# WagnerGroup/pyqmc

Measured on AMD Instinct MI355X. Metric: walker-steps/sec (VMC sweep, 64e- Slater-Jastrow), higher is better.
Workload: dtype f64

## Files before the change

### pyqmc_amd/csrc/pqa_ao.hpp

```cpp
#pragma once
#include "pqa_common.hpp"
#include "pqa_sph_high.hpp"

__device__ __forceinline__ double exp_neg(double x) {
  x = fmax(x, -800.0);
  const double k = __builtin_rint(x * 1.4426950408889634074);
  double r = fma(-k, 6.93147180369123816490e-01, x);
  r = fma(-k, 1.90821492927058770002e-10, r);
  double p = 2.519062899249436e-08;
  p = fma(p, r, 2.761249479944321e-07);
  p = fma(p, r, 2.7557019442003614e-06);
  p = fma(p, r, 2.480153911822949e-05);
  p = fma(p, r, 0.0001984127010654779);
  p = fma(p, r, 0.0013888888904182626);
  p = fma(p, r, 0.008333333333235474);
  p = fma(p, r, 0.04166666666665442);
  p = fma(p, r, 0.1666666666666677);
  p = fma(p, r, 0.5);
  p = fma(p, r, 1.0);
  p = fma(p, r, 1.0);
  return ldexp(p, (int)k);
}
__device__ __forceinline__ void exp_neg3(double x0, double x1, double x2, double& e0, double& e1, double& e2) {
  x0 = fmax(x0, -800.0); x1 = fmax(x1, -800.0); x2 = fmax(x2, -800.0);
// ... 35 lines not shown
#define SH_F3 0.5900435899266435
#define SH_F2 2.890611442640554
#define SH_F1 0.4570457994644658
#define SH_F0 0.3731763325901154
#define SH_F2C 1.445305721320277

__device__ __forceinline__ double sph_ipow(double x, int n) {
  double r = 1.0;
#pragma unroll 1
  for (int q = 0; q < n; ++q) r *= x;
  return r;
}
__device__ __forceinline__ void sph_high(int l, int m, double x, double y, double z, double& s, double& sx, double& sy, double& sz) {
  s = sx = sy = sz = 0.0;
  const int t1 = SPH_HI_OFF[l - 4][m + 1];
#pragma unroll 1
  for (int t = SPH_HI_OFF[l - 4][m]; t < t1; ++t) {
    const SphTerm q = SPH_HI_TERM[t];
    const double xa = sph_ipow(x, q.i - 1), ya = sph_ipow(y, q.j - 1), za = sph_ipow(z, q.k - 1);
    const double xi = q.i ? xa * x : 1.0, yj = q.j ? ya * y : 1.0, zk = q.k ? za * z : 1.0;
    s += q.c * xi * yj * zk;
    if (q.i) sx += q.c * q.i * xa * yj * zk;
    if (q.j) sy += q.c * q.j * xi * ya * zk;
    if (q.k) sz += q.c * q.k * xi * yj * za;
  }
}

#define PQA_RT_X0 0.0078125
#define PQA_RT_NSUB 8
#define PQA_RT_DEG 9
#define PQA_RT_REC (PQA_RT_DEG + 1)
#define PQA_RT_MINP 3
#define PQA_RT_MAXERR 2e-15
__device__ __forceinline__ double radial_tab(const double* __restrict__ tab, int nint, double r2) {
  const double y = r2 + PQA_RT_X0;
  const int E = __builtin_amdgcn_frexp_exp(y);
  const double m = __builtin_amdgcn_frexp_mant(y);
  const double t = fma(m, 2.0 * PQA_RT_NSUB, -(double)PQA_RT_NSUB);
  const double tj = floor(t);
  const double u = fma(t - tj, 2.0, -1.0);
  int idx = (E + 6) * PQA_RT_NSUB + (int)tj;
  const bool in = idx < nint;
  idx = in ? idx : nint - 1;
  const double2* rec = reinterpret_cast<const double2*>(tab + (size_t)idx * PQA_RT_REC);
  double c[PQA_RT_REC];
#pragma unroll
  for (int q = 0; q < PQA_RT_REC / 2; ++q) { const double2 v = rec[q]; c[2 * q] = v.x; c[2 * q + 1] = v.y; }
  double f0 = c[PQA_RT_DEG];
#pragma unroll
  for (int q = PQA_RT_DEG - 1; q >= 0; --q) f0 = fma(f0, u, c[q]);
  return in ? f0 : 0.0;
}
template <int NCOMP, int LMAX = 5, class Sink>
__device__ __forceinline__ void shell_angular(int l, double x, double y, double z, double R, double dRs, double lapR, Sink&& sink);
template <int NCOMP, int LMAX = 5, bool SCREEN = false, class Sink>
__device__ __forceinline__ void shell_eval(int l, double x, double y, double z, const double* __restrict__ pexp,
                                           const double* __restrict__ pcoef, int np, Sink&& sink) {
  const double r2 = x * x + y * y + z * z;
  double R = 0.0, dRs = 0.0, lapR = 0.0;
#pragma unroll 1
  for (int p = 0; p < np; ++p) {
    const double a = pexp[p];
    if (SCREEN && a * r2 > PQA_PRIM_CUT) continue;
    const double t = pcoef[p] * exp_neg(-a * r2);
    R += t;
    if (NCOMP > 1) dRs += a * t;
    if (NCOMP == 5) lapR += t * (2.0 * a) * (2.0 * a * r2 - 3.0);
  }
  shell_angular<NCOMP, LMAX>(l, x, y, z, R, dRs, lapR, sink);
}
template <int LMAX = 5, class Sink>
__device__ __forceinline__ void shell_eval_tab(int l, double x, double y, double z, const double* __restrict__ tab, int nint, Sink&& sink) {
  shell_angular<1, LMAX>(l, x, y, z, radial_tab(tab, nint, x * x + y * y + z * z), 0.0, 0.0, sink);
}
template <int NCOMP, int LMAX = 5, class Sink>
__device__ __forceinline__ void shell_eval3(int l, double x, double y, double z, const double* __restrict__ pexp,
                                            const double* __restrict__ pcoef, int np, Sink&& sink) {
  const double r2 = x * x + y * y + z * z;
  double R = 0.0, dRs = 0.0, lapR = 0.0;
  auto add = [&](double a, double c, double e) __attribute__((always_inline)) {
    const double t = c * e;
    R += t;
    if (NCOMP > 1) dRs += a * t;
    if (NCOMP == 5) lapR += t * (2.0 * a) * (2.0 * a * r2 - 3.0);
// ... 459 lines not shown
  const double* a = ao + ((size_t)c * P + p) * nao;
  double s = 0.0;
  for (int k = 0; k < nao; ++k) s += a[k] * C[(size_t)k * nmo + j];
  out[(sel ? (size_t)(sel[p] ^ 1) * slot_stride : (size_t)0) + ((size_t)p * ncomp + c) * nmo + j] = s;
}

template <int PQA_UNIT = 0>
static __global__ void k_mo_valu(const double* __restrict__ ao, const double* __restrict__ C, long rows, int nao, int nmo,
                          double* __restrict__ out) {
  const long idx = (long)blockIdx.x * blockDim.x + threadIdx.x;
  if (idx >= rows * nmo) return;
  const long r = idx / nmo;
  const int j = idx % nmo;
  double s = 0.0;
  for (int a = 0; a < nao; ++a) s += ao[r * nao + a] * C[(long)a * nmo + j];
  out[idx] = s;
}

struct ChunkTab {
  int nchunk;
  const int* chunk_nk;
  const int* shell_kb;
  const int* chunk_row0;
  const int* cw_off[3];
  const int* cw_shell[3];
  const double* cpad[2];
  int ldc[2];
  int col0;
  const double* pbc_d0;
  const unsigned long long* pbc_list;
  int pbc_nw;
  const unsigned char* out_sel;
  long out_slot_stride;
};
__device__ __forceinline__ double* orb_out(const ChunkTab& T, double* out, long p) {
  return T.out_sel ? out + (size_t)(T.out_sel[p] ^ 1) * T.out_slot_stride : out;
}

#define PQA_LS_MAX 128
#define PQA_WS_MAXSH 160
#define PQA_WS_MAXP 640

template <int NCOMP, int NT, int KC, int TP, bool LDSTAB, int PBC = 0>
static __global__ __launch_bounds__(256) void k_orb(SysDev S, ChunkTab T, int spin, PointAddr pa, long P,
                                             double* __restrict__ out) {
  P = point_count(pa, P);
  if ((long)blockIdx.x * TP >= P) return;
  constexpr int G = 256 / TP;
  constexpr int NU = (TP == 64) ? NT : ((TP == 32) ? (NT + 1) / 2 : (NT + 3) / 4);
  constexpr int KS = KC / 4;
  __shared__ double tile[NCOMP][KC][TP];
  __shared__ double sh_xyz[LDSTAB ? PQA_WS_MAXSH : 1][3];
  __shared__ int sh_meta[LDSTAB ? PQA_WS_MAXSH : 1][7];
  __shared__ double pr_exp[LDSTAB ? PQA_WS_MAXP : 1], pr_coef[LDSTAB ? PQA_WS_MAXP : 1];
  __shared__ double sh_Ls[PBC ? PQA_LS_MAX : 1][3], sh_ph[PBC == 2 ? PQA_LS_MAX : 1][2];
  const int tid = threadIdx.x, lane = tid & 63, wv = tid >> 6;
  const bool ls_lds = PBC && S.nL <= PQA_LS_MAX;
  if (PBC && ls_lds) {
    for (int q = tid; q < 3 * S.nL; q += 256) sh_Ls[q / 3][q % 3] = S.pb->Ls[q];
    if (PBC == 2) for (int q = tid; q < 2 * S.nL; q += 256) sh_ph[q / 2][q % 2] = S.pb->img_phase[q];
    if (!LDSTAB) __syncthreads();
  }
  if (LDSTAB) {
    for (int sh = tid; sh < S.nshell; sh += 256) {
      const int ia = S.shell_atom[sh];
      sh_xyz[sh][0] = S.atom_xyz[3 * ia]; sh_xyz[sh][1] = S.atom_xyz[3 * ia + 1]; sh_xyz[sh][2] = S.atom_xyz[3 * ia + 2];
// ... 413 lines not shown
```

### pyqmc_amd/csrc/pqa_create.hip

```cpp
#include "pqa_internal.hpp"

static thread_local std::string g_create_error;

static double det3(const double* a) { return a[0] * (a[4] * a[8] - a[5] * a[7]) - a[1] * (a[3] * a[8] - a[5] * a[6]) + a[2] * (a[3] * a[7] - a[4] * a[6]); }
static void inv3(const double* a, double det, double* v) {
  const double id = 1.0 / det;
  v[0] = (a[4] * a[8] - a[5] * a[7]) * id; v[1] = (a[2] * a[7] - a[1] * a[8]) * id; v[2] = (a[1] * a[5] - a[2] * a[4]) * id;
  v[3] = (a[5] * a[6] - a[3] * a[8]) * id; v[4] = (a[0] * a[8] - a[2] * a[6]) * id; v[5] = (a[2] * a[3] - a[0] * a[5]) * id;
  v[6] = (a[3] * a[7] - a[4] * a[6]) * id; v[7] = (a[1] * a[6] - a[0] * a[7]) * id; v[8] = (a[0] * a[4] - a[1] * a[3]) * id;
}

static int member_masks(pqa_handle* h, const pqa_system_t* sys, PbcDev& P) {
  P.memb_mask = nullptr;
  P.memb_E = 0;
  const int side = 2 * sys->member_M + 1, E = side, T = side + 2 * E, nc = sys->n_member_class, nj = std::min(sys->nL, 128);
  if ((size_t)nc * T * T * T * 16 > ((size_t)64 << 20)) return 0;
  std::vector<unsigned char> mem((size_t)nc * side * side * side);
  std::vector<int> imgn((size_t)sys->nL * 3);
  HIPCHK(hipMemcpy(mem.data(), sys->member, mem.size(), hipMemcpyDefault));
  HIPCHK(hipMemcpy(imgn.data(), sys->img_n, imgn.size() * sizeof(int), hipMemcpyDefault));
  for (int j = 0; j < nj; ++j)
    for (int c = 0; c < 3; ++c)
      if (std::abs(imgn[3 * j + c]) > E) return 0;
  std::vector<unsigned long long> mask((size_t)nc * T * T * T * 2, 0ull);
// ... 264 lines not shown
      c.cw_off[0].push_back((int)c.cw_shell[0].size());
    }
    std::stable_sort(members.begin(), members.end(), [&](int a, int b) { return cost(a) > cost(b); });
    std::vector<std::vector<int>> l8(8);
    std::vector<int> load8(8, 0);
    for (int s : members) {
      int best = 0;
      for (int q = 1; q < 8; ++q)
        if (load8[q] < load8[best]) best = q;
      l8[best].push_back(s);
      load8[best] += cost(s);
    }
    for (int q = 0; q < 8; ++q) {
      for (int s : l8[q]) c.cw_shell[1].push_back(s);
      c.cw_off[1].push_back((int)c.cw_shell[1].size());
    }
    std::vector<std::vector<int>> l16(16);
    std::vector<int> load16(16, 0);
    for (int s : members) {
      int best = 0;
      for (int q = 1; q < 16; ++q)
        if (load16[q] < load16[best]) best = q;
      l16[best].push_back(s);
      load16[best] += cost(s);
    }
    for (int q = 0; q < 16; ++q) {
      for (int s : l16[q]) c.cw_shell[2].push_back(s);
      c.cw_off[2].push_back((int)c.cw_shell[2].size());
    }
  }
  c.rows_pad = row0;
}

static int upload_cpad(pqa_handle* h, int t, int s, const double* mo_host) {
  const ChunkHost& c = h->chunks[t];
  const int ldc = 16 * h->nt[s], nmo = h->nmo[s];
  std::vector<double> pad((size_t)std::max(c.rows_pad, 1) * ldc, 0.0);
  for (int sh = 0; sh < h->nshell; ++sh)
    for (int m = 0; m < 2 * h->shell_l[sh] + 1; ++m)
      for (int j = 0; j < nmo; ++j)
        pad[(size_t)(c.row0[c.shell_chunk[sh]] + c.shell_kb[sh] + m) * ldc + j] = mo_host[(size_t)(h->shell_ao[sh] + m) * nmo + j];
  if (h->twist) {
    const int nr = nmo / 2;
    for (int sh = 0; sh < h->nshell; ++sh) {
      const int sx = sh + h->nshell;
      for (int m = 0; m < 2 * h->shell_l[sh] + 1; ++m)
        for (int j = 0; j < nr; ++j) {
          const double* src = mo_host + (size_t)(h->shell_ao[sh] + m) * nmo;
          double* dst = pad.data() + (size_t)(c.row0[c.shell_chunk[sx]] + c.shell_kb[sx] + m) * ldc;
          dst[j] = -src[nr + j];
          dst[nr + j] = src[j];
        }
    }
  }
  HIPCHK(hipMemcpy(h->d_cpad[t][s], pad.data(), pad.size() * sizeof(double), hipMemcpyHostToDevice));
  return 0;
}

int set_mo(pqa_handle* h, int s, const double* mo_host) {
  if (h->nmo[s] == 0 || !mo_host) return 0;
  HIPCHK(hipMemcpy(h->d_mo[s], mo_host, (size_t)h->nao * std::max(h->nmo[s], 1) * sizeof(double), hipMemcpyHostToDevice));
  for (int t = 0; t < 2; ++t) TRY(upload_cpad(h, t, s, mo_host));
  TRY(cres_upload(h, s, mo_host));
  return 0;
}

// ... 213 lines not shown
      if (!(fabs(det) > 1e-12)) FAIL("singular primitive lattice");
      inv3(a, det, P.lprim_inv);
      const size_t side = 2 * (size_t)sys->member_M + 1;
      unsigned char* tmp_b;
      TRY(upload_table(h, sys->member, (size_t)sys->n_member_class * side * side * side, &tmp_b)); P.member = tmp_b;
      TRY(upload_table(h, sys->member_class, (size_t)h->natom, &tmp_i)); P.member_class = tmp_i;
      TRY(upload_table(h, sys->img_n, (size_t)sys->nL * 3, &tmp_i)); P.img_n = tmp_i;
      TRY(upload_table(h, sys->atom_n, (size_t)h->natom * 3, &tmp_i)); P.atom_n = tmp_i;
      P.member_M = sys->member_M;
      TRY(member_masks(h, sys, P));
      for (int i = 0; i < 9; ++i) {
        double v_ = 0.0;
        for (int k = 0; k < 3; ++k) v_ += sys->lattice[3 * (i / 3) + k] * P.lprim_inv[3 * k + (i % 3)];
        P.supercell[i] = (int)lround(v_);
        if (fabs(v_ - P.supercell[i]) > 1e-6) FAIL("lattice is not an integer multiple of lattice_prim");
      }
    }
  }
  return 0;
}

static int create_determinants(pqa_handle* h, const pqa_system_t* sys) {
  SysDev& S = h->S;
  int* tmp_i;
  h->nmo[0] = sys->nmo_up; h->nmo[1] = sys->nmo_dn;
  h->ndet = sys->ndet; h->ndet_s[0] = sys->ndet_up; h->ndet_s[1] = sys->ndet_dn;
  S.ndet = h->ndet;
  const int* occ_src[2] = {sys->det_occ_up, sys->det_occ_dn};
  const double* mo_src[2] = {sys->mo_up, sys->mo_dn};
  const int nel[2] = {h->nup, h->ndn};
  shell_costs(h, sys);
  build_chunks(h, 16, h->chunks[0]);
  build_chunks(h, 32, h->chunks[1]);
  for (int s = 0; s < 2; ++s) {
    if (h->nmo[s] > (h->cplx ? 2 : 1) * PQA_MAXN) FAIL("more than 128 orbitals per spin are not supported");
    const int nt = (h->nmo[s] + 15) / 16;
    h->nt[s] = nt <= 1 ? 1 : (nt == 2 ? 2 : (nt <= 4 ? 4 : (nt <= 8 ? 8 : 16)));
    S.nmo[s] = h->nmo[s]; S.ndet_s[s] = h->ndet_s[s];
    TRY(upload_table(h, occ_src[s], (size_t)h->ndet_s[s] * nel[s], &tmp_i)); S.det_occ[s] = tmp_i;
    {
      std::vector<int> oc((size_t)std::max(nel[s], 1));
      if (nel[s] > 0) HIPCHK(hipMemcpy(oc.data(), occ_src[s], (size_t)nel[s] * sizeof(int), hipMemcpyDefault));
      S.occ_ident[s] = 1;
      for (int k = 0; k < nel[s]; ++k) S.occ_ident[s] &= (oc[k] == k) ? 1 : 0;
    }
    {
      std::vector<int> occ_h((size_t)h->ndet_s[s] * nel[s]), cm((size_t)h->ndet_s[s] * std::max(h->nmo[s], 1), -1);
      if (!occ_h.empty()) HIPCHK(hipMemcpy(occ_h.data(), occ_src[s], occ_h.size() * sizeof(int), hipMemcpyDefault));
      for (int u = 0; u < h->ndet_s[s]; ++u)
        for (int k = 0; k < nel[s]; ++k) {
          const int m = occ_h[(size_t)u * nel[s] + k];
          if (m < 0 || m >= h->nmo[s]) FAIL("determinant occupation outside the orbital range");
          cm[(size_t)u * h->nmo[s] + m] = k;
        }
      TRY(upload_table(h, cm.data(), cm.size(), &h->d_colmap[s]));
    }
    TRY(upload_table<double>(h, nullptr, (size_t)h->nao * std::max(h->nmo[s], 1), &h->d_mo[s])); S.mo[s] = h->d_mo[s];
    for (int t = 0; t < 2; ++t)
      TRY(upload_table<double>(h, nullptr, (size_t)(std::max(h->chunks[t].rows_pad, 1) + 32) * 16 * h->nt[s], &h->d_cpad[t][s]));
    if (h->nmo[s] > 0) TRY(set_mo(h, s, mo_src[s]));
  }
  TRY(upload_table(h, sys->det_coeff, (size_t)h->ndet, &h->d_detcoeff)); S.det_coeff = h->d_detcoeff;
  TRY(upload_table(h, sys->det_map, (size_t)2 * h->ndet, &tmp_i)); S.det_map = tmp_i;
  for (int t = 0; t < 2; ++t) {
    const ChunkHost& c = h->chunks[t];
    ChunkTab& T = h->tab[t];
// ... 256 lines not shown
```

### pyqmc_amd/csrc/pqa_ecp_orbcol.hpp

```cpp
#pragma once
#include "pqa_ao.hpp"
#include "pqa_ecp.hpp"

#define PQA_OC_R 16
#define PQA_OC_KC 32
#define PQA_OC_STATIC_LDS ((size_t)PQA_WS_MAXSH * (3 * sizeof(double) + 6 * sizeof(int)) + (size_t)PQA_WS_MAXP * 2 * sizeof(double) + 4 * 64 * sizeof(double) + 2 * 64 * sizeof(int))
__host__ __device__ inline size_t ecp_orbcol_lds(int nao, int n) { return (size_t)PQA_OC_R * ((size_t)(nao | 1) + (size_t)((n + PQA_OC_KC - 1) / PQA_OC_KC * PQA_OC_KC)) * sizeof(double); }

static __global__ __launch_bounds__(256) void k_ecp_orbcol(SysDev S, LwState L, ChunkTab T, int s, PointAddr pa, long P, const int* __restrict__ pte,
                                                    const int* __restrict__ ptw, long W, double* __restrict__ ratio) {
  P = point_count(pa, P);
  const long p0 = (long)blockIdx.x * 64;
  if (p0 >= P) return;
  extern __shared__ __align__(16) double oc_lds[];
  __shared__ double sh_xyz[PQA_WS_MAXSH][3];
  __shared__ int sh_meta[PQA_WS_MAXSH][6];
  __shared__ double pr_exp[PQA_WS_MAXP], pr_coef[PQA_WS_MAXP];
  __shared__ double part[4][64];
  __shared__ int run_i[64], run_w[64];
  const int tid = threadIdx.x, lane = tid & 63, wv = __builtin_amdgcn_readfirstlane(tid >> 6);
  const int n = s ? S.ndn : S.nup, nmo = S.nmo[s], nao = S.nao, vs = nao | 1, nk = (n + PQA_OC_KC - 1) / PQA_OC_KC * PQA_OC_KC;
  const int* __restrict__ occ = S.det_occ[s];
  const bool ident = S.occ_ident[s] != 0;
  const double* __restrict__ Cs = S.mo[s];
  double c[PQA_OC_KC];
  auto load_row = [&](int mu, int k0) {
    const double* __restrict__ crow = Cs + (size_t)mu * nmo;
    if (ident && (nmo & 3) == 0 && k0 + PQA_OC_KC <= n) {
#pragma unroll
      for (int u = 0; u < PQA_OC_KC; u += 4) {
        const double4 q = *reinterpret_cast<const double4*>(crow + k0 + u);
        c[u] = q.x; c[u + 1] = q.y; c[u + 2] = q.z; c[u + 3] = q.w;
      }
    } else {
#pragma unroll
      for (int u = 0; u < PQA_OC_KC; ++u) {
        const int k = k0 + u;
        c[u] = (k < n) ? crow[ident ? k : occ[k]] : 0.0;
      }
    }
  };
  bool have_c = tid < nao;
  if (have_c) load_row(tid, 0);
  const bool c_stays = nao <= 256 && n <= PQA_OC_KC;
  for (int sh = tid; sh < S.nshell; sh += 256) {
    const int ia = S.shell_atom[sh];
    sh_xyz[sh][0] = S.atom_xyz[3 * ia]; sh_xyz[sh][1] = S.atom_xyz[3 * ia + 1]; sh_xyz[sh][2] = S.atom_xyz[3 * ia + 2];
    sh_meta[sh][0] = S.shell_l[sh];
    sh_meta[sh][1] = S.shell_prim_off[sh + 1] - S.shell_prim_off[sh];
    sh_meta[sh][2] = S.shell_prim_off[sh];
    sh_meta[sh][3] = S.shell_ao_off[sh];
    sh_meta[sh][4] = S.shell_rt[2 * sh]; sh_meta[sh][5] = S.shell_rt[2 * sh + 1];
  }
  for (int p = tid; p < S.nprim; p += 256) { pr_exp[p] = S.prim_exp[p]; pr_coef[p] = S.prim_coef[p]; }
  const long pmine = (p0 + lane < P) ? p0 + lane : P - 1;
  double px, py, pz;
  load_point(pa, pmine, px, py, pz);
  const int e = pte[pmine], w = ptw[pmine];
  const int e_prev = __shfl_up(e, 1, 64), w_prev = __shfl_up(w, 1, 64);
  const bool head = lane == 0 || e != e_prev || w != w_prev;
  const unsigned long long heads = __ballot(head);
  const int run = __popcll(heads & (~0ull >> (63 - lane))) - 1, nrun = __popcll(heads);
  if (wv == 0 && head) { run_i[run] = e - s * S.nup; run_w[run] = w; }
  double* V = oc_lds;
  double* tc = oc_lds + (size_t)PQA_OC_R * vs;
  const double* __restrict__ Tt = L.Tt[s];
  const int* __restrict__ cw_off = T.cw_off[0];
  const int* __restrict__ cw_shell = T.cw_shell[0];
  double acc = 0.0;
  for (int r0 = 0; r0 < nrun; r0 += PQA_OC_R) {
    const int nr = (nrun - r0 < PQA_OC_R) ? nrun - r0 : PQA_OC_R;
    __syncthreads();
    for (int idx = tid; idx < nk * PQA_OC_R; idx += 256) {
      const int k = idx / PQA_OC_R, r = idx % PQA_OC_R;
      tc[idx] = (r < nr && k < n) ? Tt[((size_t)run_i[r0 + r] * n + k) * W + run_w[r0 + r]] : 0.0;
    }
    __syncthreads();
    for (int mu = tid; mu < nao; mu += 256) {
      double v[PQA_OC_R];
#pragma unroll
      for (int r = 0; r < PQA_OC_R; ++r) v[r] = 0.0;
      for (int k0 = 0; k0 < nk; k0 += PQA_OC_KC) {
        if (!(have_c && mu == tid && k0 == 0)) load_row(mu, k0);
        if (!c_stays) have_c = false;
#pragma unroll
        for (int g = 0; g < PQA_OC_R; g += 4) {
          if (g < nr) {
#pragma unroll
            for (int u = 0; u < PQA_OC_KC; ++u) {
              const double4 t = *reinterpret_cast<const double4*>(tc + (k0 + u) * PQA_OC_R + g);
              v[g] = fma(c[u], t.x, v[g]); v[g + 1] = fma(c[u], t.y, v[g + 1]); v[g + 2] = fma(c[u], t.z, v[g + 2]); v[g + 3] = fma(c[u], t.w, v[g + 3]);
            }
          }
        }
      }
#pragma unroll
      for (int g = 0; g < PQA_OC_R; g += 4)
        if (g < nr) { V[g * vs + mu] = v[g]; V[(g + 1) * vs + mu] = v[g + 1]; V[(g + 2) * vs + mu] = v[g + 2]; V[(g + 3) * vs + mu] = v[g + 3]; }
    }
    __syncthreads();
    const bool mine = run >= r0 && run < r0 + nr;
    const double* __restrict__ Vr = V + (mine ? run - r0 : 0) * vs;
    double a = 0.0;
    for (int ch = 0; ch < T.nchunk; ++ch) {
      const int s_end = cw_off[ch * 4 + wv + 1];
      for (int si = cw_off[ch * 4 + wv]; si < s_end; ++si) {
        const int sh = cw_shell[si];
        const int l_ = __builtin_amdgcn_readfirstlane(sh_meta[sh][0]), np_ = __builtin_amdgcn_readfirstlane(sh_meta[sh][1]);
        const int q0 = __builtin_amdgcn_readfirstlane(sh_meta[sh][2]), row = __builtin_amdgcn_readfirstlane(sh_meta[sh][3]);
        const int rt_ = __builtin_amdgcn_readfirstlane(sh_meta[sh][4]), rn_ = __builtin_amdgcn_readfirstlane(sh_meta[sh][5]);
        const double x = px - sh_xyz[sh][0], y = py - sh_xyz[sh][1], z = pz - sh_xyz[sh][2];
        auto to_sum = [&](int m, double v, double, double, double, double) { a = fma(v, Vr[row + m], a); };
        if (rt_ >= 0) shell_eval_tab(l_, x, y, z, S.rtab + rt_, rn_, to_sum);
        else shell_eval<1>(l_, x, y, z, pr_exp + q0, pr_coef + q0, np_, to_sum);
      }
    }
    if (mine) acc = a;
  }
  part[wv][lane] = acc;
  __syncthreads();
  if (wv == 0 && p0 + lane < P) ratio[p0 + lane] = ((part[0][lane] + part[1][lane]) + part[2][lane]) + part[3][lane];
}
```

### pyqmc_amd/csrc/pqa_energy.hip

```cpp
#include "pqa_internal.hpp"
#include "pqa_ecp_orbcol.hpp"

namespace {

struct EnergyPlan {
  long W = 0;
  bool soa = false;
  bool has_jastrow = false, has_j2 = false;
  bool rot_tape = false, unif_tape = false;
  enum Kinetic { kin_lw, kin_coulomb } kinetic = kin_coulomb;
  bool kin_quad = false;
  int waves = 1;
  enum Coords { coords_none, coords_sweep, coords_transpose, coords_state } coords = coords_none;
  bool soa_T = false;
  bool ewald_planes = false;
  bool ecp = false;
  enum Lists { lists_none, lists_batched, lists_lds, lists_first } lists = lists_none;
  long nseg = 1;
  size_t tab_b = 0;
  long pmax = 0;
  bool scan_small = true;
  bool fill_ue = false;
  enum Orbitals { orb_none, orb_column, orb_rows } orbitals = orb_none;
  enum Points { pts_none, pts_point_lw, pts_point, pts_accum } points = pts_none;
// ... 270 lines not shown
    TRY(ensure(h, h->b_eptw[s], n * sizeof(int)));
    TRY(ensure(h, h->b_econ[s], (h->cplx ? 2 : 1) * n * sizeof(double)));
    TRY(ensure(h, h->b_eu0[s], n * sizeof(double)));
    B.ptw[s] = (int*)h->b_eptw[s].p;
    B.u0[s] = (double*)h->b_eu0[s].p;
    if (P.orbitals == EnergyPlan::orb_column) TRY(ensure(h, h->b_erat[s], n * sizeof(double)));
    else TRY(ensure(h, h->b_emo[s], n * std::max(h->nmo[s], 1) * sizeof(double)));
    B.pts[s] = (double*)h->b_epts[s].p; B.wgt[s] = (double*)h->b_ewgt[s].p; B.pte[s] = (int*)h->b_epte[s].p;
  }
  if (batched) {
    launch_ecpb_fill(h, B, A, W);
    TRY(check_launch(h, "k_ecpb_fill"));
  }
  if (P.soa) TRY(R.side.join());
  if (batched || R.tot[0] + R.tot[1] <= 0) return 0;
  if (P.lists == EnergyPlan::lists_lds)
    hipLaunchKernelGGL(ecp_fill_t_kernels[ix(P.fill_ue)][ix(h->S.pbc)], dim3((unsigned)((W + PQA_ECP_WB - 1) / PQA_ECP_WB)), dim3(64 * PQA_ECP_WB), P.tab_b,
                       h->stream, h->S, h->js, B, h->ecp_nchan, h->ecp_nterm, W);
  else
    hipLaunchKernelGGL(ecp_fill_kernels[ix(h->S.pbc)], dim3((unsigned)W), dim3(64), 0, h->stream, h->S, h->js, B, W);
  return check_launch(h, P.lists == EnergyPlan::lists_lds ? "k_ecp_fill_t" : "k_ecp_fill");
}

int stage_ecp_orbitals(EnergyRun& R) {
  pqa_handle* h = R.h;
  const EnergyPlan& P = R.P;
  if (R.tot[0] + R.tot[1] <= 0 || P.orbitals == EnergyPlan::orb_none) return 0;
  for (int s = 0; s < 2; ++s) {
    PointAddr pa = plain_points(R.B.pts[s], R.tot[s]);
    if (P.defer) pa.count = R.cnt_dev[s];
    if (P.orbitals == EnergyPlan::orb_column) {
      if (R.tot[s] <= 0 || h->nmo[s] == 0) continue;
      hipLaunchKernelGGL((k_ecp_orbcol), dim3((unsigned)((R.tot[s] + 63) / 64)), dim3(256), ecp_orbcol_lds(h->S.nao, s ? h->ndn : h->nup), h->stream,
                         h->S, lw_state(h), h->tab[1], s, pa, R.tot[s], (const int*)R.B.pte[s], (const int*)R.B.ptw[s], P.W, (double*)h->b_erat[s].p);
    } else {
      if (P.defer) h->orb_p_hint = std::max<long>(h->en.hint[s], 1);
      const int rc = launch_orb(h, s, pa, R.tot[s], 1, (double*)h->b_emo[s].p);
      h->orb_p_hint = 0;
      if (rc != 0) return rc;
    }
  }
  return P.orbitals == EnergyPlan::orb_column ? check_launch(h, "k_ecp_orbcol") : 0;
}

using EcpAccumKernel = void (*)(SysDev, SlaterState, JastrowState, EcpBuf, int, int, const double*, const double*, long, double*, int);
using EcpPointLwKernel = void (*)(SysDev, LwState, EcpBuf, int, int, int, const double*, long, long, double*, const double*, long, double*, const double*, const double*);
using EcpPointKernel = void (*)(SysDev, SlaterState, JastrowState, EcpBuf, int, int, int, const double*, long, double*, const double*, long, long, long);
const EcpAccumKernel ecp_accum_cx_kernels[2][2] = {
    {k_ecp_accum<true, true, 4>, k_ecp_accum<true, true, 1>}, {k_ecp_accum<false, true, 4>, k_ecp_accum<false, true, 1>}};
const EcpPointLwKernel ecp_point_lw_kernels[2][2] = {
    {k_ecp_point_lw<true, true>, k_ecp_point_lw<false, true>}, {k_ecp_point_lw<true, false>, k_ecp_point_lw<false, false>}};
const EcpPointKernel ecp_point_kernels[2] = {k_ecp_point<true>, k_ecp_point<false>};

int ecp_points(EnergyRun& R) {
  pqa_handle* h = R.h;
  const EnergyPlan& P = R.P;
  const EcpBuf& B = R.B;
  const long W = P.W;
  const long* tot = R.tot;
  const bool lw = P.points == EnergyPlan::pts_point_lw, column = P.orbitals == EnergyPlan::orb_column;
  const bool both = lw && tot[0] > 0 && tot[1] > 0 && std::max(h->en.hint[0], h->en.hint[1]) <= 262144 && h->en.hint_valid;
  for (int s = 0; s < 2; ++s) {
    if (tot[s] <= 0 || (both && s == 1)) continue;
    const int o = both ? 1 : s;
    const long n = both ? std::max(tot[0], tot[1]) : tot[s];
    const dim3 g((unsigned)((n + 255) / 256), both ? 2 : 1);
    if (lw)
// ... 165 lines not shown
    if (lds <= 64 * 1024) {
      int* dgi;
      TRY(upload_table(h, gi.data(), gi.size(), &dgi));
      h->ew.gn = dgi; h->ew.nmax = nmax;
      HIPCHK(hipMemcpy(h->ew.recip, recip, 9 * sizeof(double), hipMemcpyDefault));
    }
  }
  h->ii_energy = ii;
  h->ew_set = true;
  return 0;
}

extern "C" int pqa_get_wrap(pqa_handle_t* h, int32_t* wrap) {
  HIPCHK(hipSetDevice(h->device));
  if (!h->S.pbc) FAIL("open-boundary handle has no wrap counters");
  if (h->wrap_W != h->W || h->W == 0) FAIL("no fused sweep has run on the resident walkers");
  return copy_out(h, wrap, h->b_wrap.p, (size_t)h->W * h->N * 3 * sizeof(int));
}

extern "C" int pqa_energy(pqa_handle_t* h, double threshold, const double* rot, const double* unif, uint64_t seed, double* out) {
  TRY(sync_aos(h));
  HIPCHK(hipSetDevice(h->device));
  if (h->W == 0) FAIL("state not initialised (call pqa_wf_recompute)");
  h->saved_valid = false;
  TRY(energy_dev(h, threshold, rot, unif, seed, 0u));
  return copy_out(h, out, h->b_en.p, (size_t)(h->cplx ? 7 : 6) * h->W * sizeof(double));
}

extern "C" int pqa_energy_last(pqa_handle_t* h, double* out) {
  HIPCHK(hipSetDevice(h->device));
  if (h->W == 0 || h->en.W != h->W) FAIL("no energy evaluation has run on the resident walkers");
  return copy_out(h, out, h->b_en.p, (size_t)(h->cplx ? 7 : 6) * h->W * sizeof(double));
}
```

### pyqmc_amd/csrc/pqa_internal.hpp

```cpp
#pragma once
#include <hip/hip_runtime.h>

#include <algorithm>
#include <array>
#include <cmath>
#include <cstdio>
#include <cstdlib>
#include <cstring>
#include <string>
#include <vector>

#include "../../include/pyqmc_amd.h"
#include "pqa_ao.hpp"
#include "pqa_common.hpp"
#include "pqa_cslater.hpp"
#include "pqa_dmc.hpp"
#include "pqa_energy.hpp"
#include "pqa_ecp.hpp"
#include "pqa_ecpb.hpp"
#include "pqa_jastrow.hpp"
#include "pqa_lw.hpp"
#include "pqa_slater.hpp"
#include "pqa_res.hpp"
#include "pqa_res8_tab.hpp"
// ... 30 lines not shown
  std::vector<hipEvent_t> events;
  std::vector<hipStream_t> streams;
  std::vector<void*> pinned;
  int natom = 0, nup = 0, ndn = 0, N = 0, nao = 0, nshell = 0;
  int nmo[2] = {0, 0}, nt[2] = {1, 1}, ndet = 1, ndet_s[2] = {1, 1};
  int na = 0, nb = 0, necp = 0;
  bool aos_stale = false;
  int pbc_maxcls = PQA_PRE_NCUT;
  int pbc_nw = 2;
  bool orb_general = false;
  bool dmc_continue = false, dmc_old_valid = false;
  long dmc_old_W = 0;
  bool invert_attr = false;
  bool big = false;
  bool pbc_high_l = false;
  bool twist = false;
  bool cplx = false;
  bool has_slater = false, has_jastrow = false;
  bool has_j2 = false, has_j3 = false;
  int na3 = 0, nb3 = 0;
  double* d_c3 = nullptr;
  DevBuf b_j3u;
  double ii_energy = 0.0;
  EwaldDev ew{};
  bool ew_set = false;
  std::vector<int> shell_l, shell_np, shell_ao;
  int lmax = 0;
  std::vector<int> rt_shells;
  double rt_err = 0.0;
  std::vector<int> shell_cost;
  SysDev S{};
  ChunkHost chunks[2];
  ChunkTab tab[2]{};
  const unsigned char* out_sel = nullptr;
  long out_slot_stride = 0;
  int orb_col0 = 0;
  double* d_mo[2] = {nullptr, nullptr};
  double* d_cpad[2][2] = {{nullptr, nullptr}, {nullptr, nullptr}};
  double *d_acoeff = nullptr, *d_bcoeff = nullptr, *d_detcoeff = nullptr, *d_quad = nullptr, *d_quadw = nullptr;
  int *d_ecp_naip = nullptr, *d_ecp_qoff = nullptr;
  int ecp_naip = 0;
  std::vector<int> ecp_nch;
  int ecpb_on = 0, ecpb_npoints = 0, ecpb_nsd = 0, ecpb_nsr = 0, ecpb_nsel = 0;
  int *d_ecpb_naip = nullptr, *d_ecpb_qoff = nullptr, *d_ecpb_pstart = nullptr;
  double *d_aq = nullptr, *d_bq = nullptr;
  int jas_merge = 1;
  long W = 0;
  SlaterState st{};
  JastrowState js{};
  DevBuf b_x, b_T[2], b_dsign[2], b_dlog[2], b_cache[2], b_aval, b_bval;
  DevBuf b_alt_x, b_alt_T[2], b_alt_dsign[2], b_alt_dlog[2], b_alt_cache[2], b_alt_aval, b_alt_bval, b_alt_j3u, b_rsidx;
  DevBuf b_pts, b_motmp, b_out, b_widx, b_mask, b_ao, b_flag, b_newpos, b_aux, b_accept, b_accrec, b_acccnt, b_accw, b_dwrap, b_wrap, b_epass, b_eptw[2], b_econ[2], b_eu0[2], b_tves, b_pgdet, b_pbcd0, b_pbcmask, b_pbcth, b_tmuold;
  int* d_colmap[2] = {nullptr, nullptr};
  int jas_fold_allowed = 1;
  int ecp_nchan = 0, ecp_nterm = 0;
  long wrap_W = 0;
  DevBuf b_gauss, b_unif, b_kc, b_en, b_means, b_sign, b_log, b_ju;
  DevBuf b_orbphi[2];
  DevBuf b_s2out;
  DevBuf b_tbpts;
  DevBuf b_j3dm;
  DevBuf b_symx, b_symdet[2], b_symout;
  DevBuf b_sqq, b_sqout, b_sqpart, b_sqacc;
  DevBuf b_e2tab, b_e2out, b_e2acc;
  DevBuf b_gps_par, b_gps_x, b_gps_e, b_gps_s;
  int gps_nsup = 0;
// ... 274 lines not shown
```

Before: 3.246 million.

## Precompute per-wave shell program for ECP orbital-column kernel and prefetch radial tables

Builds a host-side per-wave list of shell records (centre, l, primitive offset, AO row, radial-table index) that the ECP orbital-column kernel reads through constant-address loads, replacing the per-block LDS staging of shell metadata. The radial-table lookup is split into a request and a finish step so the next shell's coefficients are fetched while the current shell's angular part is evaluated. The first batch of T-column values is gathered before the main loop, with primitive loading interleaved, and each wave keeps its own run indices. Occupancy is hinted with launch bounds (256, 3), and optional clock probes are added behind a macro. The cost is more live registers from the software pipeline and an extra device table.

Result: no change. 3.274 million, median of 6 (+0.8%).

```diff
diff --git a/pyqmc_amd/csrc/pqa_ao.hpp b/pyqmc_amd/csrc/pqa_ao.hpp
--- a/pyqmc_amd/csrc/pqa_ao.hpp
+++ b/pyqmc_amd/csrc/pqa_ao.hpp
@@ -91,24 +91,35 @@
 #define PQA_RT_REC (PQA_RT_DEG + 1)
 #define PQA_RT_MINP 3
 #define PQA_RT_MAXERR 2e-15
-__device__ __forceinline__ double radial_tab(const double* __restrict__ tab, int nint, double r2) {
+struct RadialReq {
+  double u;
+  bool in;
+  double c[PQA_RT_REC];
+};
+__device__ __forceinline__ RadialReq radial_tab_request(const double* __restrict__ tab, int nint, double r2) {
+  RadialReq q;
   const double y = r2 + PQA_RT_X0;
   const int E = __builtin_amdgcn_frexp_exp(y);
   const double m = __builtin_amdgcn_frexp_mant(y);
   const double t = fma(m, 2.0 * PQA_RT_NSUB, -(double)PQA_RT_NSUB);
   const double tj = floor(t);
-  const double u = fma(t - tj, 2.0, -1.0);
+  q.u = fma(t - tj, 2.0, -1.0);
   int idx = (E + 6) * PQA_RT_NSUB + (int)tj;
-  const bool in = idx < nint;
-  idx = in ? idx : nint - 1;
+  q.in = idx < nint;
+  idx = q.in ? idx : nint - 1;
   const double2* rec = reinterpret_cast<const double2*>(tab + (size_t)idx * PQA_RT_REC);
-  double c[PQA_RT_REC];
-#pragma unroll
-  for (int q = 0; q < PQA_RT_REC / 2; ++q) { const double2 v = rec[q]; c[2 * q] = v.x; c[2 * q + 1] = v.y; }
-  double f0 = c[PQA_RT_DEG];
-#pragma unroll
-  for (int q = PQA_RT_DEG - 1; q >= 0; --q) f0 = fma(f0, u, c[q]);
-  return in ? f0 : 0.0;
+#pragma unroll
+  for (int k = 0; k < PQA_RT_REC / 2; ++k) { const double2 v = rec[k]; q.c[2 * k] = v.x; q.c[2 * k + 1] = v.y; }
+  return q;
+}
+__device__ __forceinline__ double radial_tab_finish(const RadialReq& q) {
+  double f0 = q.c[PQA_RT_DEG];
+#pragma unroll
+  for (int k = PQA_RT_DEG - 1; k >= 0; --k) f0 = fma(f0, q.u, q.c[k]);
+  return q.in ? f0 : 0.0;
+}
+__device__ __forceinline__ double radial_tab(const double* __restrict__ tab, int nint, double r2) {
+  return radial_tab_finish(radial_tab_request(tab, nint, r2));
 }
 template <int NCOMP, int LMAX = 5, class Sink>
 __device__ __forceinline__ void shell_angular(int l, double x, double y, double z, double R, double dRs, double lapR, Sink&& sink);
@@ -634,6 +645,16 @@
   int pbc_nw;
   const unsigned char* out_sel;
   long out_slot_stride;
+};
+struct OcShell {
+  int l, np, q0, row;
+  int rt, rn;
+  int pad[2];
+  double x, y, z, pad2;
+};
+struct OcTab {
+  const OcShell* shell;
+  int off[5];
 };
 __device__ __forceinline__ double* orb_out(const ChunkTab& T, double* out, long p) {
   return T.out_sel ? out + (size_t)(T.out_sel[p] ^ 1) * T.out_slot_stride : out;
diff --git a/pyqmc_amd/csrc/pqa_create.hip b/pyqmc_amd/csrc/pqa_create.hip
--- a/pyqmc_amd/csrc/pqa_create.hip
+++ b/pyqmc_amd/csrc/pqa_create.hip
@@ -320,6 +320,29 @@
   c.rows_pad = row0;
 }
 
+static int build_orbcol_program(pqa_handle* h, const pqa_system_t* sys) {
+  const ChunkHost& c = h->chunks[1];
+  std::vector<OcShell> rec;
+  for (int g = 0; g < 4; ++g) {
+    h->oc.off[g] = (int)rec.size();
+    for (int ch = 0; ch < (int)c.nk.size(); ++ch)
+      for (int si = c.cw_off[0][ch * 4 + g]; si < c.cw_off[0][ch * 4 + g + 1]; ++si) {
+        const int sh = c.cw_shell[0][si];
+        OcShell r{};
+        const double* centre = sys->atom_xyz + 3 * sys->shell_atom[sh];
+        r.l = h->shell_l[sh]; r.np = h->shell_np[sh]; r.q0 = sys->shell_prim_off[sh]; r.row = h->shell_ao[sh];
+        r.rt = h->rt_shells[2 * sh]; r.rn = h->rt_shells[2 * sh + 1];
+        r.x = centre[0]; r.y = centre[1]; r.z = centre[2];
+        rec.push_back(r);
+      }
+  }
+  h->oc.off[4] = (int)rec.size();
+  rec.push_back(OcShell{});
+  OcShell* d = nullptr;
+  TRY(upload_table(h, rec.data(), rec.size(), &d)); h->oc.shell = d;
+  return 0;
+}
+
 static int upload_cpad(pqa_handle* h, int t, int s, const double* mo_host) {
   const ChunkHost& c = h->chunks[t];
   const int ldc = 16 * h->nt[s], nmo = h->nmo[s];
@@ -599,6 +622,7 @@
   shell_costs(h, sys);
   build_chunks(h, 16, h->chunks[0]);
   build_chunks(h, 32, h->chunks[1]);
+  TRY(build_orbcol_program(h, sys));
   for (int s = 0; s < 2; ++s) {
     if (h->nmo[s] > (h->cplx ? 2 : 1) * PQA_MAXN) FAIL("more than 128 orbitals per spin are not supported");
     const int nt = (h->nmo[s] + 15) / 16;
diff --git a/pyqmc_amd/csrc/pqa_ecp_orbcol.hpp b/pyqmc_amd/csrc/pqa_ecp_orbcol.hpp
--- a/pyqmc_amd/csrc/pqa_ecp_orbcol.hpp
+++ b/pyqmc_amd/csrc/pqa_ecp_orbcol.hpp
@@ -7,17 +7,34 @@
 #define PQA_OC_STATIC_LDS ((size_t)PQA_WS_MAXSH * (3 * sizeof(double) + 6 * sizeof(int)) + (size_t)PQA_WS_MAXP * 2 * sizeof(double) + 4 * 64 * sizeof(double) + 2 * 64 * sizeof(int))
 __host__ __device__ inline size_t ecp_orbcol_lds(int nao, int n) { return (size_t)PQA_OC_R * ((size_t)(nao | 1) + (size_t)((n + PQA_OC_KC - 1) / PQA_OC_KC * PQA_OC_KC)) * sizeof(double); }
 
-static __global__ __launch_bounds__(256) void k_ecp_orbcol(SysDev S, LwState L, ChunkTab T, int s, PointAddr pa, long P, const int* __restrict__ pte,
-                                                    const int* __restrict__ ptw, long W, double* __restrict__ ratio) {
+__device__ __forceinline__ OcShell oc_record(const OcShell* tab, int j) {
+  typedef __attribute__((address_space(4))) const int* ci_ptr;
+  typedef __attribute__((address_space(4))) const double* cd_ptr;
+  const ci_ptr qi = (ci_ptr)(tab + j);
+  const cd_ptr qd = (cd_ptr)(tab + j);
+  OcShell r;
+  r.l = qi[0]; r.np = qi[1]; r.q0 = qi[2]; r.row = qi[3]; r.rt = qi[4]; r.rn = qi[5];
+  r.x = qd[4]; r.y = qd[5]; r.z = qd[6];
+  return r;
+}
+
+#ifdef PQA_OC_CLK
+static __device__ unsigned long long pqa_oc_clk[64 * 8];
+#define PQA_OCCLK(k) do { if (blockIdx.x < 64 && threadIdx.x == 0) pqa_oc_clk[blockIdx.x * 8 + (k)] = wall_clock64(); } while (0)
+#else
+#define PQA_OCCLK(k) do { } while (0)
+#endif
+
+static __global__ __launch_bounds__(256, 3) void k_ecp_orbcol(SysDev S, LwState L, OcTab O, int s, PointAddr pa, long P, const int* __restrict__ pte,
+                                                       const int* __restrict__ ptw, long W, double* __restrict__ ratio) {
   P = point_count(pa, P);
   const long p0 = (long)blockIdx.x * 64;
   if (p0 >= P) return;
+  PQA_OCCLK(0);
   extern __shared__ __align__(16) double oc_lds[];
-  __shared__ double sh_xyz[PQA_WS_MAXSH][3];
-  __shared__ int sh_meta[PQA_WS_MAXSH][6];
   __shared__ double pr_exp[PQA_WS_MAXP], pr_coef[PQA_WS_MAXP];
   __shared__ double part[4][64];
-  __shared__ int run_i[64], run_w[64];
+  __shared__ int run_i[4][64], run_w[4][64];
   const int tid = threadIdx.x, lane = tid & 63, wv = __builtin_amdgcn_readfirstlane(tid >> 6);
   const int n = s ? S.ndn : S.nup, nmo = S.nmo[s], nao = S.nao, vs = nao | 1, nk = (n + PQA_OC_KC - 1) / PQA_OC_KC * PQA_OC_KC;
   const int* __restrict__ occ = S.det_occ[s];
@@ -42,17 +59,6 @@
   };
   bool have_c = tid < nao;
   if (have_c) load_row(tid, 0);
-  const bool c_stays = nao <= 256 && n <= PQA_OC_KC;
-  for (int sh = tid; sh < S.nshell; sh += 256) {
-    const int ia = S.shell_atom[sh];
-    sh_xyz[sh][0] = S.atom_xyz[3 * ia]; sh_xyz[sh][1] = S.atom_xyz[3 * ia + 1]; sh_xyz[sh][2] = S.atom_xyz[3 * ia + 2];
-    sh_meta[sh][0] = S.shell_l[sh];
-    sh_meta[sh][1] = S.shell_prim_off[sh + 1] - S.shell_prim_off[sh];
-    sh_meta[sh][2] = S.shell_prim_off[sh];
-    sh_meta[sh][3] = S.shell_ao_off[sh];
-    sh_meta[sh][4] = S.shell_rt[2 * sh]; sh_meta[sh][5] = S.shell_rt[2 * sh + 1];
-  }
-  for (int p = tid; p < S.nprim; p += 256) { pr_exp[p] = S.prim_exp[p]; pr_coef[p] = S.prim_coef[p]; }
   const long pmine = (p0 + lane < P) ? p0 + lane : P - 1;
   double px, py, pz;
   load_point(pa, pmine, px, py, pz);
@@ -61,28 +67,45 @@
   const bool head = lane == 0 || e != e_prev || w != w_prev;
   const unsigned long long heads = __ballot(head);
   const int run = __popcll(heads & (~0ull >> (63 - lane))) - 1, nrun = __popcll(heads);
-  if (wv == 0 && head) { run_i[run] = e - s * S.nup; run_w[run] = w; }
+  if (head) { run_i[wv][run] = e - s * S.nup; run_w[wv][run] = w; }
+  __builtin_amdgcn_fence(__ATOMIC_ACQ_REL, "wavefront");
+  __builtin_amdgcn_wave_barrier();
   double* V = oc_lds;
   double* tc = oc_lds + (size_t)PQA_OC_R * vs;
   const double* __restrict__ Tt = L.Tt[s];
-  const int* __restrict__ cw_off = T.cw_off[0];
-  const int* __restrict__ cw_shell = T.cw_shell[0];
+  {
+    const int r = tid % PQA_OC_R, kq = tid / PQA_OC_R, nr = nrun < PQA_OC_R ? nrun : PQA_OC_R;
+    const bool rin = r < nr;
+    const double* __restrict__ col = Tt + (size_t)run_i[wv][rin ? r : 0] * n * W + run_w[wv][rin ? r : 0];
+    for (int k0 = 0; k0 < nk; k0 += 2 * PQA_OC_R) {
+      const int ka = k0 + kq, kb = ka + PQA_OC_R;
+      const double ta = col[(size_t)(ka < n ? ka : 0) * W], tb = col[(size_t)(kb < n ? kb : 0) * W];
+      if (k0 == 0)
+        for (int p = tid; p < S.nprim; p += 256) { pr_exp[p] = S.prim_exp[p]; pr_coef[p] = S.prim_coef[p]; }
+      tc[ka * PQA_OC_R + r] = (rin && ka < n) ? ta : 0.0;
+      tc[kb * PQA_OC_R + r] = (rin && kb < n) ? tb : 0.0;
+    }
+  }
+  PQA_OCCLK(2);
   double acc = 0.0;
   for (int r0 = 0; r0 < nrun; r0 += PQA_OC_R) {
     const int nr = (nrun - r0 < PQA_OC_R) ? nrun - r0 : PQA_OC_R;
-    __syncthreads();
-    for (int idx = tid; idx < nk * PQA_OC_R; idx += 256) {
-      const int k = idx / PQA_OC_R, r = idx % PQA_OC_R;
-      tc[idx] = (r < nr && k < n) ? Tt[((size_t)run_i[r0 + r] * n + k) * W + run_w[r0 + r]] : 0.0;
+    if (r0 > 0) {
+      __syncthreads();
+      for (int idx = tid; idx < nk * PQA_OC_R; idx += 256) {
+        const int k = idx / PQA_OC_R, r = idx % PQA_OC_R;
+        tc[idx] = (r < nr && k < n) ? Tt[((size_t)run_i[wv][r0 + r] * n + k) * W + run_w[wv][r0 + r]] : 0.0;
+      }
     }
     __syncthreads();
+    if (r0 == 0) PQA_OCCLK(1);
     for (int mu = tid; mu < nao; mu += 256) {
       double v[PQA_OC_R];
 #pragma unroll
       for (int r = 0; r < PQA_OC_R; ++r) v[r] = 0.0;
       for (int k0 = 0; k0 < nk; k0 += PQA_OC_KC) {
         if (!(have_c && mu == tid && k0 == 0)) load_row(mu, k0);
-        if (!c_stays) have_c = false;
+        have_c = false;
 #pragma unroll
         for (int g = 0; g < PQA_OC_R; g += 4) {
           if (g < nr) {
@@ -99,25 +122,32 @@
         if (g < nr) { V[g * vs + mu] = v[g]; V[(g + 1) * vs + mu] = v[g + 1]; V[(g + 2) * vs + mu] = v[g + 2]; V[(g + 3) * vs + mu] = v[g + 3]; }
     }
     __syncthreads();
+    if (r0 == 0) PQA_OCCLK(3);
     const bool mine = run >= r0 && run < r0 + nr;
     const double* __restrict__ Vr = V + (mine ? run - r0 : 0) * vs;
     double a = 0.0;
-    for (int ch = 0; ch < T.nchunk; ++ch) {
-      const int s_end = cw_off[ch * 4 + wv + 1];
-      for (int si = cw_off[ch * 4 + wv]; si < s_end; ++si) {
-        const int sh = cw_shell[si];
-        const int l_ = __builtin_amdgcn_readfirstlane(sh_meta[sh][0]), np_ = __builtin_amdgcn_readfirstlane(sh_meta[sh][1]);
-        const int q0 = __builtin_amdgcn_readfirstlane(sh_meta[sh][2]), row = __builtin_amdgcn_readfirstlane(sh_meta[sh][3]);
-        const int rt_ = __builtin_amdgcn_readfirstlane(sh_meta[sh][4]), rn_ = __builtin_amdgcn_readfirstlane(sh_meta[sh][5]);
-        const double x = px - sh_xyz[sh][0], y = py - sh_xyz[sh][1], z = pz - sh_xyz[sh][2];
-        auto to_sum = [&](int m, double v, double, double, double, double) { a = fma(v, Vr[row + m], a); };
-        if (rt_ >= 0) shell_eval_tab(l_, x, y, z, S.rtab + rt_, rn_, to_sum);
-        else shell_eval<1>(l_, x, y, z, pr_exp + q0, pr_coef + q0, np_, to_sum);
+    const int j0 = __builtin_amdgcn_readfirstlane(O.off[wv]), j1 = __builtin_amdgcn_readfirstlane(O.off[wv + 1]);
+    auto to_sum_at = [&](int row) { return [&a, Vr, row](int m, double v, double, double, double, double) { a = fma(v, Vr[row + m], a); }; };
+    if (j0 < j1) {
+      OcShell cur = oc_record(O.shell, j0), nxt = oc_record(O.shell, min(j0 + 1, j1 - 1));
+      double x = px - cur.x, y = py - cur.y, z = pz - cur.z;
+      RadialReq rq = {};
+      if (cur.rt >= 0) rq = radial_tab_request(S.rtab + cur.rt, cur.rn, x * x + y * y + z * z);
+      for (int j = j0; j < j1; ++j) {
+        const OcShell nx2 = oc_record(O.shell, min(j + 2, j1 - 1));
+        const double nx = px - nxt.x, ny = py - nxt.y, nz = pz - nxt.z;
+        const double R = cur.rt >= 0 ? radial_tab_finish(rq) : 0.0;
+        if (nxt.rt >= 0) rq = radial_tab_request(S.rtab + nxt.rt, nxt.rn, nx * nx + ny * ny + nz * nz);
+        if (cur.rt >= 0) shell_angular<1>(cur.l, x, y, z, R, 0.0, 0.0, to_sum_at(cur.row));
+        else shell_eval<1>(cur.l, x, y, z, pr_exp + cur.q0, pr_coef + cur.q0, cur.np, to_sum_at(cur.row));
+        cur = nxt; nxt = nx2; x = nx; y = ny; z = nz;
       }
     }
     if (mine) acc = a;
   }
   part[wv][lane] = acc;
+  PQA_OCCLK(4);
   __syncthreads();
   if (wv == 0 && p0 + lane < P) ratio[p0 + lane] = ((part[0][lane] + part[1][lane]) + part[2][lane]) + part[3][lane];
+  PQA_OCCLK(5);
 }
diff --git a/pyqmc_amd/csrc/pqa_energy.hip b/pyqmc_amd/csrc/pqa_energy.hip
--- a/pyqmc_amd/csrc/pqa_energy.hip
+++ b/pyqmc_amd/csrc/pqa_energy.hip
@@ -326,7 +326,7 @@
     if (P.orbitals == EnergyPlan::orb_column) {
       if (R.tot[s] <= 0 || h->nmo[s] == 0) continue;
       hipLaunchKernelGGL((k_ecp_orbcol), dim3((unsigned)((R.tot[s] + 63) / 64)), dim3(256), ecp_orbcol_lds(h->S.nao, s ? h->ndn : h->nup), h->stream,
-                         h->S, lw_state(h), h->tab[1], s, pa, R.tot[s], (const int*)R.B.pte[s], (const int*)R.B.ptw[s], P.W, (double*)h->b_erat[s].p);
+                         h->S, lw_state(h), h->oc, s, pa, R.tot[s], (const int*)R.B.pte[s], (const int*)R.B.ptw[s], P.W, (double*)h->b_erat[s].p);
     } else {
       if (P.defer) h->orb_p_hint = std::max<long>(h->en.hint[s], 1);
       const int rc = launch_orb(h, s, pa, R.tot[s], 1, (double*)h->b_emo[s].p);
@@ -558,3 +558,9 @@
   if (h->W == 0 || h->en.W != h->W) FAIL("no energy evaluation has run on the resident walkers");
   return copy_out(h, out, h->b_en.p, (size_t)(h->cplx ? 7 : 6) * h->W * sizeof(double));
 }
+
+#ifdef PQA_OC_CLK
+extern "C" int pqa_debug_oc_clk(unsigned long long* dst, int n) {
+  return (int)hipMemcpyFromSymbol(dst, HIP_SYMBOL(pqa_oc_clk), (size_t)n * sizeof(unsigned long long));
+}
+#endif
diff --git a/pyqmc_amd/csrc/pqa_internal.hpp b/pyqmc_amd/csrc/pqa_internal.hpp
--- a/pyqmc_amd/csrc/pqa_internal.hpp
+++ b/pyqmc_amd/csrc/pqa_internal.hpp
@@ -86,6 +86,7 @@
   SysDev S{};
   ChunkHost chunks[2];
   ChunkTab tab[2]{};
+  OcTab oc{};
   const unsigned char* out_sel = nullptr;
   long out_slot_stride = 0;
   int orb_col0 = 0;
```
